# elrodrigues/deneva-plus

Measured on AMD Instinct MI355X. Metric: committed txns/sec (node) YCSB zipf0.9 at 1/2/4/8 GPUs; abort-set bit-exact, higher is better.
Workload: dtype u64; 1 GPU; YCSB config D: 16,777,216 rows/partition, 1,048,576-txn epoch in total; cc_alg=NO_WAIT, rows_per_partition=16777216, txns_per_epoch=1048576, txns_per_epoch_per_gpu=1048576, req_per_query=10, parallelism=1 GPU, decision_lanes=4, sequence_order=one origin

## Files before the change

deneva-plus_amd/csrc/dvcc_common.h:

```cpp
#pragma once
#include "dvcc_internal.h"

namespace dvcc {

__device__ __forceinline__ uint32_t mask_rank(uint64_t mask) {
    return __builtin_amdgcn_mbcnt_hi((uint32_t)(mask >> 32),
                                     __builtin_amdgcn_mbcnt_lo((uint32_t)mask, 0u));
}

__device__ __forceinline__ uint64_t match_digit(uint32_t d, uint64_t valid) {
    uint64_t peers = valid;
#pragma unroll
    for (int b = 0; b < kRadixBits; b++) {
        const uint32_t bit = (d >> b) & 1u;
        const uint64_t m = __ballot(bit);
        peers &= bit ? m : ~m;
    }
    return peers;
}

__device__ __forceinline__ uint32_t block_excl_scan256(uint32_t v, uint32_t *lds4, uint32_t *total) {
    const uint32_t lane = threadIdx.x & 63, wave = threadIdx.x >> 6;
    uint32_t x = v;
#pragma unroll
// ... 256 lines not shown
    } else {
        for (uint32_t j = t.bstart[bk], end = t.bstart[bk + 1]; j < end; j++) {
            const IxEntry e = t.ix[j];
            if (e.key == key) { row = e.row; found = true; break; }
        }
    }
    if (!found) {
        if (miss) *miss = true;
        else set_err(ctr, ERRB_KEY);
    }
    row += t.row_base;
    return found;
}

template <bool DENSE>
__device__ __forceinline__ bool kk_row(const KillKeys &kk, uint64_t key, uint64_t &row, Counters *ctr) {
    if constexpr (DENSE) {
        row = key + kk.dense_base;
        if (key < kk.dense_lim) return true;
        set_err(ctr, ERRB_KEY);
        return false;
    } else {
        return probe_row(kk.tabs.t[0], kk.tabs.n > 0, key, row, ctr);
    }
}

__device__ __forceinline__ uint32_t row_word(const uint32_t *__restrict__ acc_row, const RecRows &rr, uint64_t a) {
    if (rr.on && !rr.recs)
        return (uint32_t)(rr.keys[a] + rr.dense_base) | (rr.types[a] == DV_WR ? AR_WR : 0u);
    const uint32_t w = (rr.on ? rr.recs : acc_row)[a];
    return ((w & ~AR_WR) + (rr.on ? (uint32_t)rr.dense_base : 0u)) | (w & AR_WR);
}

}
```

deneva-plus_amd/csrc/dvcc_kernels.hip:

```cpp
#include <hip/hip_ext.h>

#include "dvcc_common.h"
#include "dvcc_tpcc.h"

#ifndef DVCC_PROBE_HIST_WAVES
#define DVCC_PROBE_HIST_WAVES 6
#endif

namespace dvcc {


constexpr int kPV = 4;
template <bool HIST, bool RSV>
__device__ __forceinline__ void probe_body(const Tables &tabs, const uint64_t *__restrict__ keys,
                                           const uint32_t *__restrict__ keys32,
                                                  const uint8_t *__restrict__ types,
                                                  const uint32_t *__restrict__ acc_txn,
                                                  const uint8_t *__restrict__ tables, uint64_t n,
                                                  uint32_t n_txn, uint32_t slog,
                                                  uint64_t *__restrict__ pairs,
                                                  uint32_t *__restrict__ tb_start,
                                                  uint32_t *__restrict__ tb_end,
                                                  uint8_t *__restrict__ tlen,
                                                  uint32_t *__restrict__ acc_row, Counters *ctr,
// ... 271 lines not shown
                              acc_txn, tables, n_acc, n_txn, slog, pairs, tb_start, tb_end, tlen, acc_row, ctr,
                              counts, ntiles, ts, rsv_cols);
    else if (counts)
        DV_LAUNCH_EV(k_probe_hist<false>, blocks, kBlock, 0, s, ev0, ev1, tabs, keys, keys32, types,
                              acc_txn, tables, n_acc, n_txn, slog, pairs, tb_start, tb_end, tlen, acc_row, ctr,
                              counts, ntiles, ts, nullptr);
    else if (rsv_cols)
        DV_LAUNCH_EV(k_probe<true>, blocks, kBlock, 0, s, ev0, ev1, tabs, keys, keys32, types, acc_txn,
                              tables, n_acc, n_txn, slog, pairs, tb_start, tb_end, tlen, acc_row, ctr, lim, ts, n_dev,
                              rsv_cols);
    else
        DV_LAUNCH_EV(k_probe<false>, blocks, kBlock, 0, s, ev0, ev1, tabs, keys, keys32, types, acc_txn,
                              tables, n_acc, n_txn, slog, pairs, tb_start, tb_end, tlen, acc_row, ctr, lim, ts, n_dev,
                              nullptr);
}

__global__ __launch_bounds__(kBlock) void k_probe_tb(Tables tabs, const uint64_t *__restrict__ keys,
                                                     const uint8_t *__restrict__ types,
                                                     const uint32_t *__restrict__ recs,
                                                     const uint32_t *__restrict__ txn_begin, uint64_t n_acc,
                                                     uint32_t n_txn, uint32_t K, uint32_t slog,
                                                     uint64_t *__restrict__ pairs, uint8_t *__restrict__ tlen,
                                                     uint32_t *__restrict__ acc_row, Counters *ctr,
                                                     const uint64_t *__restrict__ ts,
                                                     const uint32_t *__restrict__ n_acc_dev) {
    if (n_acc_dev && (uint64_t)*n_acc_dev < n_acc) n_acc = *n_acc_dev;
    if (blockIdx.x == 0 && threadIdx.x == 0) {
        ctr->n_acc = (uint32_t)n_acc;
        const uint64_t ak = txn_begin[K];
        ctr->a_acc = (uint32_t)(ak < n_acc ? ak : n_acc);
        if (txn_begin[0] != 0u || txn_begin[n_txn] != n_acc) set_err(ctr, ERRB_TXN);
    }
    bool bad = false, big_seen = false, ts_bad = false;
    for (uint32_t t = blockIdx.x * kBlock + threadIdx.x; t < n_txn; t += gridDim.x * kBlock) {
        const uint32_t a0 = txn_begin[t], a1 = txn_begin[t + 1];
        if (a1 < a0 || a1 > n_acc) {
            bad = true;
            continue;
        }
        const uint32_t len = a1 - a0;
        const bool big = len > (1u << slog);
        big_seen |= big;
        if (ts && t > 0 && ts[t] <= ts[t - 1]) ts_bad = true;
        if (t >= K) continue;
        tlen[t] = (uint8_t)(big ? (1u << slog) : len);
        constexpr uint32_t kU = 8;
        for (uint32_t j0 = 0; j0 < len; j0 += kU) {
            uint64_t key[kU];
            uint32_t wrs[kU];
            const KillKeys kk{tabs, keys, types, recs, 0, 0};
#pragma unroll
            for (uint32_t j = 0; j < kU; j++) {
                wrs[j] = 0;
                key[j] = j0 + j < len ? kk_key(kk, a0 + j0 + j, wrs[j]) : 0ull;
            }
#pragma unroll
            for (uint32_t j = 0; j < kU; j++) {
                if (j0 + j >= len) break;
                uint64_t row = 0;
                probe_row(tabs.t[0], tabs.n > 0, key[j], row, ctr);
                const uint32_t wr = wrs[j];
                const uint32_t pos = j0 + j;
                if (acc_row) acc_row[a0 + pos] = (uint32_t)row | (wr ? AR_WR : 0u);
                pairs[a0 + pos] = pair_pack(row, t, (pos >> slog) ? 0u : pos, wr);
            }
        }
    }
    if (bad) set_err(ctr, ERRB_TXN);
    if (big_seen) set_err(ctr, ERRB_BIG);
    if (ts_bad) set_err(ctr, ERRB_TS);
}

void launch_probe_tb(hipStream_t s, const Tables &tabs, const uint64_t *keys, const uint8_t *types,
                     const uint32_t *recs, const uint32_t *txn_begin, uint64_t n_acc, uint32_t n_txn, uint32_t K,
                     uint32_t slog, uint64_t *pairs, uint8_t *tlen, uint32_t *acc_row, Counters *ctr,
                     const uint64_t *ts, hipEvent_t ev0, hipEvent_t ev1, const uint32_t *n_acc_dev) {
#ifndef DVCC_PROBE_TB_GRID
#define DVCC_PROBE_TB_GRID 4096
#endif
    uint32_t g = (n_txn + kBlock - 1) / kBlock;
    g = g < 1 ? 1 : (g > DVCC_PROBE_TB_GRID ? DVCC_PROBE_TB_GRID : g);
    DV_LAUNCH_EV(k_probe_tb, g, kBlock, 0, s, ev0, ev1, tabs, keys, types, recs, txn_begin, n_acc, n_txn, K, slog,
                 pairs, tlen, acc_row, ctr, ts, n_acc_dev);
}


__device__ __forceinline__ uint64_t sort_n(uint64_t n, const uint32_t *n_dev) {
    return n_dev && (uint64_t)*n_dev < n ? (uint64_t)*n_dev : n;
}

__device__ __forceinline__ uint32_t row_hash(uint64_t key, uint32_t hmul, int hbits) {
    return ((uint32_t)(key >> 32) * hmul) & ((1u << hbits) - 1u);
}
template <int W>
__device__ __forceinline__ uint32_t key_digit(uint64_t key, int shift, uint32_t hmul, int hbits) {
    return hmul ? row_hash(key, hmul, hbits) >> (hbits - W) : (uint32_t)(key >> shift) & ((1u << W) - 1u);
}

// ... 26 lines not shown
        } else if (valid) {
            atomicAdd(&wc[wave][d], 1u);
        }
    }
    __syncthreads();
    for (uint32_t d = tid; d < kRadix; d += kBlock)
        counts[(uint64_t)d * nblocks + blockIdx.x] = wc[0][d] + wc[1][d] + wc[2][d] + wc[3][d];
}

__global__ __launch_bounds__(kBlock) void k_radix_scan(uint32_t *__restrict__ counts, uint32_t nblocks,
                                                       uint32_t *__restrict__ digit_tot,
                                                       const uint32_t *__restrict__ n_dev) {
    __shared__ uint32_t lds4[4];
    uint32_t *c = counts + (uint64_t)blockIdx.x * nblocks;
    if (n_dev && nblocks_for(*n_dev) < nblocks) nblocks = nblocks_for(*n_dev);
    const uint32_t tot = block_chunk_scan256(c, nblocks, lds4);
    if (threadIdx.x == 0) digit_tot[blockIdx.x] = tot;
}

__global__ __launch_bounds__(kBlock) void k_radix_scatter(
    const uint64_t *__restrict__ in, uint64_t *__restrict__ out, uint64_t n, int shift, const uint32_t *__restrict__ counts,
    const uint32_t *__restrict__ digit_tot, uint32_t nblocks, const uint32_t *__restrict__ n_dev,
    uint32_t hmul, int hbits, uint32_t *__restrict__ digit_pre) {
    __shared__ __attribute__((aligned(16))) uint64_t skeys[kTile];
    n = sort_n(n, n_dev);
    if ((uint64_t)blockIdx.x * kTile >= n) return;
    __shared__ uint32_t wc[4][kRadix];
    __shared__ uint32_t dstart[kRadix];
    __shared__ uint64_t gbase[kRadix];
    __shared__ uint32_t lds4[4];
    const uint32_t tid = threadIdx.x, lane = tid & 63, wave = tid >> 6;
    const uint64_t tile0 = (uint64_t)blockIdx.x * kTile;

    {
        const uint32_t d = tid;
        const uint32_t dex = block_excl_scan256(digit_tot[d], lds4, nullptr);
        if (digit_pre && blockIdx.x == 0) digit_pre[d] = dex;
        gbase[d] = (uint64_t)dex + counts[(uint64_t)d * nblocks + blockIdx.x];
        for (int w = 0; w < 4; w++) wc[w][d] = 0;
    }
    __syncthreads();

    const uint64_t base = tile0 + wave * (64 * kIPT);
    uint64_t k[kIPT];
    uint32_t r[kIPT];
#pragma unroll
    for (int j = 0; j < kIPT; j++) {
        const uint64_t idx = base + j * 64 + lane;
        k[j] = idx < n ? in[idx] : 0;
    }
#pragma unroll
    for (int j = 0; j < kIPT; j++) {
        const uint64_t idx = base + j * 64 + lane;
        const bool valid = idx < n;
        const uint32_t d = key_digit<kRadixBits>(k[j], shift, hmul, hbits);
        const uint64_t vmask = __ballot(valid);
        const uint64_t peers = match_digit(d, vmask);
        const uint32_t before = wc[wave][d];
        r[j] = before + mask_rank(peers);
        if (valid && lane == (uint32_t)__builtin_ctzll(peers)) wc[wave][d] = before + (uint32_t)__popcll(peers);
    }
    __syncthreads();
    {
        const uint32_t d = tid;
        const uint32_t c0 = wc[0][d], c1 = wc[1][d], c2 = wc[2][d], c3 = wc[3][d];
        wc[0][d] = 0;
        wc[1][d] = c0;
        wc[2][d] = c0 + c1;
        wc[3][d] = c0 + c1 + c2;
        const uint32_t ds = block_excl_scan256(c0 + c1 + c2 + c3, lds4, nullptr);
        dstart[d] = ds;
        gbase[d] -= ds;
    }
    __syncthreads();
#pragma unroll
    for (int j = 0; j < kIPT; j++) {
        const uint64_t idx = base + j * 64 + lane;
        if (idx < n) {
            const uint32_t d = key_digit<kRadixBits>(k[j], shift, hmul, hbits);
            const uint32_t pos = dstart[d] + wc[wave][d] + r[j];
            skeys[pos] = k[j];
        }
    }
    __syncthreads();
    const uint32_t tile_n = (uint32_t)((n - tile0) < (uint64_t)kTile ? (n - tile0) : kTile);
    for (uint32_t p = tid; p < tile_n; p += kBlock) {
        const uint64_t key = skeys[p];
// ... 26 lines not shown
    for (int j = 0; j < kIPT; j++) {
        const uint64_t idx = base + j * 64 + lane;
        const bool valid = idx < n;
        const uint32_t d = key_digit<W>(k[j], shift, hmul, hbits);
        const uint32_t d0 = __builtin_amdgcn_readfirstlane(d);
        const uint64_t vmask = __ballot(valid);
        if (__ballot(valid && d == d0) == vmask) {
            if (lane == 0) wc[wave][d0] += (uint32_t)__popcll(vmask);
        } else if (valid) {
            atomicAdd(&wc[wave][d], 1u);
        }
    }
    __syncthreads();
    for (uint32_t d = tid; d < R; d += kBlock)
        counts[(uint64_t)d * nblocks + blockIdx.x] = wc[0][d] + wc[1][d] + wc[2][d] + wc[3][d];
}

template <int W>
__global__ __launch_bounds__(kBlock) void k_radix_scatter_w(const uint64_t *__restrict__ in, uint64_t *__restrict__ out,
                                                            uint64_t n, int shift, const uint32_t *__restrict__ counts,
                                                            const uint32_t *__restrict__ digit_tot, uint32_t nblocks,
                                                            const uint32_t *__restrict__ n_dev, uint32_t hmul,
                                                            int hbits, uint32_t *__restrict__ digit_pre) {
    constexpr uint32_t R = 1u << W, PER = R / kBlock;
    __shared__ __attribute__((aligned(16))) uint64_t skeys[kTile];
    __shared__ uint32_t wc[4][R];
    __shared__ uint32_t dstart[R];
    __shared__ uint32_t gbase[R];
    __shared__ uint32_t lds4[4];
    n = sort_n(n, n_dev);
    if ((uint64_t)blockIdx.x * kTile >= n) return;
    const uint32_t tid = threadIdx.x, lane = tid & 63, wave = tid >> 6;
    const uint64_t tile0 = (uint64_t)blockIdx.x * kTile;
    {
        uint32_t t[PER], sum = 0;
#pragma unroll
        for (uint32_t q = 0; q < PER; q++) {
            t[q] = digit_tot[tid * PER + q];
            sum += t[q];
        }
        uint32_t pre = block_excl_scan256(sum, lds4, nullptr);
#pragma unroll
        for (uint32_t q = 0; q < PER; q++) {
            const uint32_t d = tid * PER + q;
            if (digit_pre && blockIdx.x == 0) digit_pre[d] = pre;
            gbase[d] = pre + counts[(uint64_t)d * nblocks + blockIdx.x];
            pre += t[q];
            wc[0][d] = wc[1][d] = wc[2][d] = wc[3][d] = 0;
        }
    }
    __syncthreads();
    const uint64_t base = tile0 + wave * (64 * kIPT);
    uint64_t k[kIPT];
    uint32_t r[kIPT];
#pragma unroll
    for (int j = 0; j < kIPT; j++) {
        const uint64_t idx = base + j * 64 + lane;
        k[j] = idx < n ? in[idx] : 0;
    }
#pragma unroll
    for (int j = 0; j < kIPT; j++) {
        const uint64_t idx = base + j * 64 + lane;
        const bool valid = idx < n;
        const uint32_t d = key_digit<W>(k[j], shift, hmul, hbits);
        uint64_t peers = __ballot(valid);
#pragma unroll
        for (int b = 0; b < W; b++) {
            const uint32_t bit = (d >> b) & 1u;
            const uint64_t m = __ballot(bit);
            peers &= bit ? m : ~m;
        }
        const uint32_t before = wc[wave][d];
        r[j] = before + mask_rank(peers);
        if (valid && lane == (uint32_t)__builtin_ctzll(peers)) wc[wave][d] = before + (uint32_t)__popcll(peers);
    }
    __syncthreads();
    {
        uint32_t tot[PER], sum = 0;
#pragma unroll
        for (uint32_t q = 0; q < PER; q++) {
            const uint32_t d = tid * PER + q;
            const uint32_t c0 = wc[0][d], c1 = wc[1][d], c2 = wc[2][d], c3 = wc[3][d];
            wc[0][d] = 0;
            wc[1][d] = c0;
            wc[2][d] = c0 + c1;
            wc[3][d] = c0 + c1 + c2;
            tot[q] = c0 + c1 + c2 + c3;
            sum += tot[q];
        }
        uint32_t ds = block_excl_scan256(sum, lds4, nullptr);
#pragma unroll
        for (uint32_t q = 0; q < PER; q++) {
            const uint32_t d = tid * PER + q;
            dstart[d] = ds;
            gbase[d] -= ds;
            ds += tot[q];
// ... 250 lines not shown
            const uint32_t d = valid ? ((row_hash(src[i], hmul, hbits) & hmask) >> sh) & (kRadix - 1) : 0u;
            const uint32_t d0 = __builtin_amdgcn_readfirstlane(d);
            const uint64_t vm = __ballot(valid);
            if (__ballot(valid && d == d0) == vm) {
                if (lane == 0 && vm) atomicAdd(&tot[d0], (uint32_t)__popcll(vm));
            } else if (valid) {
                atomicAdd(&tot[d], 1u);
            }
        }
        __syncthreads();
        if (tid < 64) {
            uint32_t v[4], s4 = 0;
#pragma unroll
            for (int q = 0; q < 4; q++) {
                v[q] = tot[4 * lane + q];
                s4 += v[q];
            }
            uint32_t pre = wave_incl_sum(s4, lane) - s4;
#pragma unroll
            for (int q = 0; q < 4; q++) {
                run[4 * lane + q] = pre;
                pre += v[q];
            }
        }
        __syncthreads();
        for (uint32_t c0 = 0; c0 < m; c0 += kChunk) {
            const uint32_t mc = m - c0 < kChunk ? m - c0 : kChunk;
            const uint32_t steps = (mc + kBucketThreads - 1) / kBucketThreads;
            for (uint32_t d = lane; d < (uint32_t)kRadix; d += 64) wc[wave][d] = 0;
            uint64_t k[kBucketGroup];
            uint32_t r[kBucketGroup];
#pragma unroll
            for (int s = 0; s < kBucketGroup; s++) {
                if ((uint32_t)s < steps) {
                    const uint32_t e = (wave * steps + s) * 64 + lane;
                    const bool valid = e < mc;
                    k[s] = valid ? src[c0 + e] : 0ull;
                    r[s] = bucket_rank(((row_hash(k[s], hmul, hbits) & hmask) >> sh) & (kRadix - 1), valid,
                                       wc[wave], lane);
                }
            }
            __syncthreads();
            bucket_bases(wc, tot, run);
#pragma unroll
            for (int s = 0; s < kBucketGroup; s++) {
                if ((uint32_t)s < steps) {
                    const uint32_t e = (wave * steps + s) * 64 + lane;
                    if (e < mc) dst[wc[wave][((row_hash(k[s], hmul, hbits) & hmask) >> sh) & (kRadix - 1)] + r[s]] = k[s];
                }
            }
            __syncthreads();
        }
    }
    if (!(passes & 1)) {
        for (uint32_t i = tid; i < m; i += kBucketThreads) B[i] = A[i];
    }
}

int radix_sort_rows(hipStream_t s, uint64_t *pairs[2], uint64_t n, int key_bits, uint32_t *counts,
                    uint32_t *digit_tot, hipEvent_t *scatter_ev, bool hist0_done, const uint32_t *n_dev,
                    bool lsd_only) {
    if (n == 0) return 0;
    const uint32_t nb = nblocks_for(n);
    int cur = 0, pass = 0;
    if (!lsd_only && bucket_sort_applies(n, key_bits, hist0_done, n_dev != nullptr)) {
        const int lo = kBucketLoBits(key_bits);
        const uint32_t hmul = kRowHashMul;
        uint32_t *digit_pre = digit_tot + kRadixMax;
        hipEvent_t e0 = scatter_ev ? scatter_ev[0] : nullptr, e1 = scatter_ev ? scatter_ev[1] : nullptr;
        if (lo == 9)
// ... 599 lines not shown
```

deneva-plus_amd/csrc/dvcc_prefix.hip:

```cpp
#include <algorithm>

#include "dvcc_common.h"

namespace dvcc {

namespace {
#ifndef DVCC_KILL_IPT
#define DVCC_KILL_IPT 2
#endif
constexpr int kKillIPT = DVCC_KILL_IPT;
constexpr uint32_t kKillTile = kBlock * kKillIPT;
constexpr uint32_t RS_RD = 1u, RS_WR = 2u;

__device__ __forceinline__ uint32_t row_bits(const uint32_t *rs, uint32_t row) {
    return (rs[row >> 4] >> ((row & 15u) * 2u)) & 3u;
}
}

#ifndef DVCC_HOT_LOG
#define DVCC_HOT_LOG 16
#endif
#ifndef DVCC_BLOOM_LOG
#define DVCC_BLOOM_LOG 20
#endif
constexpr uint32_t kHotRows = 1u << DVCC_HOT_LOG, kHotWords = kHotRows / 16;
constexpr uint32_t kBloomBits = 1u << DVCC_BLOOM_LOG, kBloomWords = kBloomBits / 32;
static_assert((kHotWords + kBloomWords) * sizeof(uint32_t) <= 160u * 1024u,
              "k_kill's hot row words + Bloom filter exceed gfx950's 160 KiB of LDS per workgroup");
__device__ __forceinline__ uint32_t bloom_bit(uint32_t row) { return (row * 0x9E3779B1u) >> (32 - DVCC_BLOOM_LOG); }

uint64_t row_state_words(uint64_t rows) {
    return std::max<uint64_t>(((rows + 15) / 16 + 3) & ~3ull, kHotWords) + kBloomWords;
}

#ifndef DVCC_MARK_BLOCK
#define DVCC_MARK_BLOCK 512
#endif
constexpr int kMarkBlock = DVCC_MARK_BLOCK;
__global__ __launch_bounds__(kMarkBlock) void k_prefix_mark(uint8_t *__restrict__ status,
                                                            const uint32_t *__restrict__ tb_start,
                                                            const uint32_t *__restrict__ tb_end,
                                                            const uint32_t *__restrict__ acc_row, RecRows rr,
                                                            uint32_t K, uint32_t *__restrict__ row_state,
                                                            uint64_t state_words,
                                                            uint32_t *__restrict__ bloom, int nowait,
                                                            Counters *__restrict__ ctr,
                                                            const uint32_t *__restrict__ words) {
    __shared__ uint32_t s_hot[kHotWords];
    if (input_err(ctr)) return;
    if (ctr->halt) {
        if (blockIdx.x == 0 && threadIdx.x == 0) ctr->a_halt = 1u;
        return;
    }
    if (blockIdx.x == 0 && threadIdx.x == 0) {
        const uint32_t r0 = ctr->async_wr0 ? ctr->async_wr0 : ctr->async_r0;
        ctr->a_rounds = r0 ? r0 + ctr->async_iters : 1u;
    }
    for (uint32_t i = threadIdx.x; i < kHotWords; i += kMarkBlock) s_hot[i] = 0;
    __syncthreads();
    uint32_t und = 0;
    for (uint32_t t = blockIdx.x * kMarkBlock + threadIdx.x; t < K; t += gridDim.x * kMarkBlock) {
        if (words) {
            const uint8_t st = word_status(words[t]);
            status[t] = st;
            und += st == ST_UNDEC ? 1u : 0u;
            if (st != ST_COMMIT) continue;
        } else if (status[t] != ST_COMMIT) {
            continue;
        }
        constexpr uint32_t kMU = 8;
        for (uint32_t a0 = tb_start[t], e = tb_end[t]; a0 < e; a0 += kMU) {
            uint32_t arw[kMU];
#pragma unroll
            for (uint32_t u = 0; u < kMU; u++) arw[u] = a0 + u < e ? row_word(acc_row, rr, a0 + u) : 0u;
#pragma unroll
            for (uint32_t u = 0; u < kMU; u++) {
                if (a0 + u >= e) continue;
                const uint32_t ar = arw[u];
                const uint32_t row = ar & ~AR_WR;
                const uint32_t bit = (ar & AR_WR) ? RS_WR : (nowait ? RS_RD : 0u);
                if (!bit) continue;
                if (row < kHotRows) {
                    atomicOr(&s_hot[row >> 4], bit << ((row & 15u) * 2u));
                } else {
                    atomicOr(&row_state[row >> 4], bit << ((row & 15u) * 2u));
                    const uint32_t h = bloom_bit(row);
                    atomicOr(&bloom[h >> 5], 1u << (h & 31u));
                }
            }
        }
    }
    if (und) {
        set_err(ctr, ERRB_SPIN);
        atomicMax(&ctr->spin_site, 2u);
    }
    __syncthreads();
    for (uint32_t i = threadIdx.x; i < kHotWords && i < state_words; i += kMarkBlock) {
        const uint32_t w = s_hot[i];
        if (w) atomicOr(&row_state[i], w);
    }
}

#ifndef DVCC_KILL_WORDS
#define DVCC_KILL_WORDS 8
#endif
constexpr int kKillWords = DVCC_KILL_WORDS;
constexpr int kKillBlock = 1024;
#ifndef DVCC_KILL_GRID
#define DVCC_KILL_GRID 256
// ... 208 lines not shown
        info[t - K] = killed ? 0u : len | 0x80000000u;
        cnt += killed ? 0u : 1u;
        acc += len;
    }
    uint32_t tc = 0, ta = 0;
    (void)block_excl_scan256(cnt, lds4, &tc);
    (void)block_excl_scan256(acc, lds4, &ta);
    if (tid == 0) {
        tsum[2 * blockIdx.x] = tc;
        tsum[2 * blockIdx.x + 1] = ta;
    }
}

template <int KEYS>
__global__ __launch_bounds__(kBlock) void k_kill_emit(
    const uint32_t *__restrict__ tb_start, const uint32_t *__restrict__ tb_end, uint32_t *__restrict__ acc_row,
    uint32_t K, uint32_t n_txn,
    const uint64_t *__restrict__ skip_bits, const uint32_t *__restrict__ info, const uint32_t *__restrict__ tsum,
    uint32_t *__restrict__ map,
    uint8_t *__restrict__ status_b, uint8_t *__restrict__ tlen_b, uint64_t *__restrict__ pairs_b, Counters *ctr,
    KillKeys kk, const uint32_t *__restrict__ row_state, int nowait) {
    __shared__ Agg wt_c[kBlock / 64], wt_a[kBlock / 64], wt_f[kBlock / 64];
    __shared__ uint32_t s_sub0, s_ab0, s_nsurv, s_nacc, s_nfull;
    __shared__ uint32_t l_a0[kKillTile], l_pre[kKillTile + 1];
    __shared__ uint32_t l_st[kKillTile], l_len[kKillTile];
    __shared__ uint32_t l_end[KEYS ? kKillTile : 1], l_fl[KEYS ? kKillTile : 1], l_skip[KEYS ? kKillTile : 1];
    __shared__ uint32_t l_fpre[KEYS == 1 ? kKillTile + 1 : 1];
    const uint32_t m = n_txn > K ? n_txn - K : 0u;
    const uint32_t ntiles = (m + kKillTile - 1) / kKillTile;
    if (blockIdx.x >= ntiles || input_err(ctr) || ctr->halt) return;
    const uint32_t tid = threadIdx.x, lane = tid & 63, wave = tid >> 6;
    const uint32_t tile = blockIdx.x;
    const uint32_t t_lo = K + tile * kKillTile;
#pragma unroll
    for (int j = 0; j < kKillIPT; j++) {
        const uint32_t t = t_lo + j * kBlock + tid;
        l_st[j * kBlock + tid] = t < n_txn ? tb_start[t] : 0u;
        l_len[j * kBlock + tid] = t < n_txn ? info[t - K] : 0u;
        if constexpr (KEYS) l_end[j * kBlock + tid] = t < n_txn ? tb_end[t] : 0u;
    }
    if (wave < 2) {
        uint32_t sum = 0;
        for (uint32_t q0 = 0; q0 < tile; q0 += 8 * 64) {
            uint32_t v[8];
#pragma unroll
            for (uint32_t u = 0; u < 8; u++) {
                const uint32_t q = q0 + u * 64 + lane;
                v[u] = q < tile ? tsum[2 * q + wave] : 0u;
            }
#pragma unroll
            for (uint32_t u = 0; u < 8; u++) sum += v[u];
        }
#pragma unroll
        for (int off = 32; off > 0; off >>= 1) sum += __shfl_xor(sum, off, 64);
        if (lane == 0) {
            (wave == 0 ? s_sub0 : s_ab0) = sum;
            if (tile == ntiles - 1) (wave == 0 ? ctr->b_txn : ctr->b_acc) = sum + tsum[2 * tile + wave];
        }
    }
    __syncthreads();
    const uint32_t first = t_lo + tid * kKillIPT;
    uint32_t surv = 0, cnt = 0, acc = 0, full = 0;
    uint32_t a0s[kKillIPT], lens[kKillIPT], fls[kKillIPT];
#pragma unroll
    for (int j = 0; j < kKillIPT; j++) {
        const uint32_t w = l_len[tid * kKillIPT + j];
        a0s[j] = l_st[tid * kKillIPT + j];
        lens[j] = w & 0x7FFFFFFFu;
        fls[j] = KEYS ? l_end[tid * kKillIPT + j] - a0s[j] : 0u;
        if (!w) continue;
        surv |= 1u << j;
        cnt++;
// ... 41 lines not shown
        l_a0[ls] = a0s[j];
        l_pre[ls] = la;
        if constexpr (KEYS) l_fl[ls] = fls[j];
        if constexpr (KEYS == 1) {
            l_fpre[ls] = lf;
            l_skip[ls] = 0;
        }
        if constexpr (KEYS == 2)
            l_skip[ls] = skip_bits && fls[j] <= 32u ? range_field(skip_bits, a0s[j], a0s[j] + fls[j]) : 0u;
        la += lens[j];
        lf += fls[j];
        ls++;
    }
    if (tid == 0) {
        l_pre[s_nsurv] = s_nacc;
        if constexpr (KEYS == 1) l_fpre[s_nsurv] = s_nfull;
    }
    __syncthreads();
    if constexpr (KEYS == 1) {
        constexpr uint32_t kU = 4;
        const uint32_t ns = s_nsurv, nf = s_nfull;
        for (uint32_t g0 = 0; g0 < nf; g0 += kBlock * kU) {
            uint32_t a[kU], wr[kU];
            uint64_t key[kU];
#pragma unroll
            for (uint32_t u = 0; u < kU; u++) {
                const uint32_t g = g0 + u * kBlock + tid;
                uint32_t lo = 0, hi = ns;
                while (hi - lo > 1) {
                    const uint32_t mid = (lo + hi) >> 1;
                    if (l_fpre[mid] <= g) lo = mid;
                    else hi = mid;
                }
                a[u] = l_a0[lo] + (g - l_fpre[lo]);
                wr[u] = 0;
                key[u] = g < nf ? kk_key(kk, a[u], wr[u]) : 0ull;
            }
            uint32_t rows[kU];
#pragma unroll
            for (uint32_t u = 0; u < kU; u++) {
                uint64_t row = 0;
                if (g0 + u * kBlock + tid < nf)
                    kk_row<false>(kk, key[u], row, ctr);
                rows[u] = (uint32_t)row;
            }
#pragma unroll
            for (uint32_t u = 0; u < kU; u++) {
                const uint32_t g = g0 + u * kBlock + tid;
                if (g >= nf) continue;
                acc_row[a[u]] = rows[u] | (wr[u] ? AR_WR : 0u);
#ifdef DVCC_EMIT_ROW_STATE
                const bool skip = nowait && !wr[u] && row_bits(row_state, rows[u]) == RS_RD;
#else
                const bool skip = skip_bits && ((skip_bits[a[u] >> 6] >> (a[u] & 63u)) & 1ull) != 0;
#endif
                if (skip) {
                    uint32_t lo = 0, hi = ns;
                    while (hi - lo > 1) {
                        const uint32_t mid = (lo + hi) >> 1;
                        if (l_fpre[mid] <= g) lo = mid;
                        else hi = mid;
                    }
                    if (l_fpre[lo + 1] - l_fpre[lo] <= 32u) atomicOr(&l_skip[lo], 1u << (g - l_fpre[lo]));
                }
            }
        }
        __syncthreads();
    }
    constexpr uint32_t kCompactU = 4;
    const uint32_t ns = s_nsurv, na = s_nacc, ab0 = s_ab0;
    for (uint32_t g0 = 0; g0 < na; g0 += kBlock * kCompactU) {
        uint32_t sv[kCompactU], qv[kCompactU], ar[kCompactU];
#pragma unroll
        for (uint32_t u = 0; u < kCompactU; u++) {
            const uint32_t g = g0 + u * kBlock + tid;
            uint32_t lo = 0, hi = ns;
            while (hi - lo > 1) {
                const uint32_t mid = (lo + hi) >> 1;
                if (l_pre[mid] <= g) lo = mid;
                else hi = mid;
            }
            sv[u] = lo;
            qv[u] = g - l_pre[lo];
            uint32_t a = 0;
            if (g < na) {
                if constexpr (KEYS) {
                    if (l_fl[lo] <= 32u) {
                        uint32_t kept = ~l_skip[lo];
                        for (uint32_t r = qv[u]; r; r--) kept &= kept - 1;
                        a = l_a0[lo] + (uint32_t)__builtin_ctz(kept);
                    } else {
                        a = skip_bits ? nth_kept(skip_bits, l_a0[lo], qv[u]) : l_a0[lo] + qv[u];
                    }
                } else {
                    a = skip_bits ? nth_kept(skip_bits, l_a0[lo], qv[u]) : l_a0[lo] + qv[u];
                }
            }
            if constexpr (KEYS) {
                uint64_t row = 0;
                uint32_t w = 0;
                if (g < na) kk_row<KEYS == 2>(kk, kk_key(kk, a, w), row, ctr);
                ar[u] = g < na ? (uint32_t)row | (w ? AR_WR : 0u) : 0u;
            } else {
                ar[u] = g < na ? acc_row[a] : 0u;
            }
        }
#pragma unroll
        for (uint32_t u = 0; u < kCompactU; u++) {
            const uint32_t g = g0 + u * kBlock + tid;
            if (g < na) pairs_b[ab0 + g] = pair_pack(ar[u] & ~AR_WR, sub0 + sv[u], qv[u], ar[u] >> 31);
        }
    }
}

__global__ __launch_bounds__(kBlock) void k_sub_scatter_back(const uint32_t *__restrict__ map,
                                                             const uint8_t *__restrict__ status_b,
                                                             uint8_t *__restrict__ status, Counters *ctr,
                                                             const uint32_t *__restrict__ words) {
    if (input_err(ctr) || ctr->halt) return;
    const uint32_t S = ctr->b_txn;
    uint32_t und = 0;
    for (uint32_t i = blockIdx.x * kBlock + threadIdx.x; i < S; i += gridDim.x * kBlock) {
        const uint8_t st = words ? word_status(words[i]) : status_b[i];
        status[map[i]] = st;
        und += st == ST_UNDEC ? 1u : 0u;
    }
    if (und) {
        set_err(ctr, ERRB_SPIN);
        atomicMax(&ctr->spin_site, 2u);
    }
}

namespace {
uint32_t grid_of(uint64_t n, uint32_t cap) {
    const uint64_t g = (n + kBlock - 1) / kBlock;
    return (uint32_t)(g < 1 ? 1 : (g > cap ? cap : g));
}
}
// ... 56 lines not shown
```

deneva-plus_amd/csrc/dvcc_rounds.hip:

```cpp
#include <hip/hip_ext.h>

#include "dvcc_common.h"

namespace dvcc {

namespace {

constexpr uint32_t B_CA = 1u, B_UA = 2u, B_CW = 4u, B_UW = 8u, B_KEEP = 16u;
constexpr uint32_t kCarryHead = 1u << 31;
constexpr uint32_t kCarryInit = B_UA | B_UW | B_KEEP | kCarryHead;
constexpr uint8_t VB_OK = 1, VB_ABORT = 2;
constexpr uint32_t F_WR = 1u, F_HEAD = 2u, F_DONE = 4u;

template <class E>
__device__ __forceinline__ uint32_t r_txn(E e, uint32_t slog) {
    return (uint32_t)(e >> (slog + 3));
}

template <class E>
__device__ __forceinline__ uint32_t elem_value(E e, uint8_t s, int nowait) {
    const bool wr = (e & F_WR) != 0;
    if (s == ST_COMMIT) return (nowait ? B_CA : 0u) | (wr ? B_CW : 0u);
    if (s == ST_UNDEC) return (nowait ? B_UA : 0u) | (wr ? B_UW : 0u);
    return 0u;
}

template <bool ALL = false, class E>
__device__ __forceinline__ E decide_elem(E e, uint32_t excl, int nowait, uint8_t *__restrict__ vb8,
                                         uint32_t slog, uint8_t *status) {
    if (e & F_DONE) return e;
    const uint32_t sel = (nowait && (e & F_WR)) ? (excl & (B_CA | B_UA)) : ((excl >> 2) & (B_CA | B_UA));
    if (sel & B_CA) {
        status[r_txn(e, slog)] = ST_ABORT;
// ... 113 lines not shown
#define DVCC_ROUND_T64 1024
#endif
#ifndef DVCC_ROUND_IPT64
#define DVCC_ROUND_IPT64 4
#endif
struct Geo {
    static constexpr int kThreads = sizeof(EIn) == 4 ? 1024 : DVCC_ROUND_T64;
    static constexpr int kMinWaves = sizeof(EIn) == 4 ? 4 : 3;
    static constexpr int kWaves = kThreads / 64;
    static constexpr int kIPT = sizeof(EIn) == 4 ? DVCC_ROUND_IPT : DVCC_ROUND_IPT64;
    static constexpr uint32_t kTile = kThreads * kIPT;
    static_assert(kTile >= (uint32_t)kRTile, "round tiles at least kRTile elements");
};
__device__ __forceinline__ uint32_t pad16(uint32_t j) { return j + (j >> 4); }

template <class EIn>
struct TileLds {
    EIn el[Geo<EIn>::kTile + Geo<EIn>::kTile / 16];
    EIn next;
    uint64_t prev;
    Agg wt[Geo<EIn>::kWaves];
    RAgg rw[Geo<EIn>::kWaves];
    Agg pre;
    uint32_t tot;
    uint32_t gpos;
};

template <class EIn>
__device__ __forceinline__ void load_tile(const EIn *__restrict__ src, uint32_t base, uint32_t tile_n,
                                          uint32_t n, EIn *s, EIn *s_next, EIn past_end) {
    constexpr int V = 16 / sizeof(EIn);
    constexpr int T = Geo<EIn>::kThreads;
    const uint32_t tid = threadIdx.x;
#pragma unroll
    for (int q = 0; q < Geo<EIn>::kIPT / V; q++) {
        const uint32_t j = (q * T + tid) * V;
        if (j + V <= tile_n) {
            if constexpr (V == 2) {
                const ulonglong2 x = *reinterpret_cast<const ulonglong2 *>(src + base + j);
                s[pad16(j)] = x.x;
                s[pad16(j + 1)] = x.y;
            } else {
                const uint4 x = *reinterpret_cast<const uint4 *>(src + base + j);
                s[pad16(j)] = x.x;
                s[pad16(j + 1)] = x.y;
                s[pad16(j + 2)] = x.z;
                s[pad16(j + 3)] = x.w;
            }
        } else {
            for (int k = 0; k < V; k++)
                if (j + k < tile_n) s[pad16(j + k)] = src[base + j + k];
        }
    }
    if (tid == 0) *s_next = base + tile_n < n ? src[base + tile_n] : past_end;
}

template <bool FIRST, class EIn, class E>
__device__ __forceinline__ void round_tile(TileLds<EIn> &sh, uint32_t tile, uint32_t n, uint32_t ntiles,
                                           const EIn *__restrict__ el_in, E *__restrict__ el_out,
                                           uint32_t *__restrict__ n_out, uint8_t *status,
                                           uint8_t *__restrict__ vb8, uint32_t slog, int nowait,
                                           uint64_t *desc, uint32_t tag, uint32_t *und_reset,
                                           Counters *ctr);

__device__ __forceinline__ void reset_und(uint32_t *und_reset, Counters *ctr) {
    if (und_reset) *und_reset = 0;
    else for (int k = 0; k < kSlots; k++) ctr->slot[k].undecided = 0;
}

template <bool FIRST, class EIn, class E>
__device__ __forceinline__ void round_tile(TileLds<EIn> &sh, uint32_t tile, uint32_t n, uint32_t ntiles,
                                           const EIn *__restrict__ el_in, E *__restrict__ el_out,
                                           uint32_t *__restrict__ n_out, uint8_t *status,
                                           uint8_t *__restrict__ vb8, uint32_t slog, int nowait,
                                           uint64_t *desc, uint32_t tag, uint32_t *und_reset,
                                           Counters *ctr) {
    using G = Geo<EIn>;
    constexpr int IPT = G::kIPT;
    const uint32_t tid = threadIdx.x, lane = tid & 63, wave = tid >> 6;
    const uint32_t base = tile * G::kTile;
    const uint32_t tile_n = n - base < G::kTile ? n - base : G::kTile;
    load_tile<EIn>(el_in, base, tile_n, n, sh.el, &sh.next, FIRST ? (EIn)~0ull : (EIn)F_HEAD);
    if (FIRST && tid == 0) sh.prev = base > 0 ? (uint64_t)el_in[base - 1] : ~0ull;
    __syncthreads();

    const uint32_t first = tid * IPT;
    const int cnt = first >= tile_n ? 0 : (tile_n - first < (uint32_t)IPT ? (int)(tile_n - first) : IPT);
    E e[IPT];
    uint32_t v[IPT];
    uint32_t nhm = 0;
    uint32_t tmask = 0;
    if constexpr (FIRST) {
        uint64_t pp = first == 0 ? sh.prev : (uint64_t)sh.el[pad16(first - 1)];
        const uint64_t pn = first + IPT < tile_n ? (uint64_t)sh.el[pad16(first + IPT)] : (uint64_t)sh.next;
        uint64_t p[IPT];
#pragma unroll
        for (int j = 0; j < IPT; j++) p[j] = j < cnt ? (uint64_t)sh.el[pad16(first + j)] : ~0ull;
#pragma unroll
        for (int j = 0; j < IPT; j++) {
            e[j] = (E)F_HEAD;
            if (j < cnt) {
                const bool head = pair_row(pp) != pair_row(p[j]);
                const uint64_t q = j + 1 < cnt ? p[j + 1] : (cnt < IPT ? ~0ull : pn);
                const bool rep = !head && pair_txn(pp) == pair_txn(p[j]);
                uint32_t wr = (uint32_t)(p[j] & 1u);
                const uint64_t id = ((uint64_t)pair_txn(p[j]) << slog) | pair_pos(p[j]);
                if (rep) {
                    tmask |= 1u << j;
                    vb8[id] = VB_OK;
                    if (nowait && ((p[j] | pp) & 1u)) status[pair_txn(p[j])] = ST_ABORT;
                } else if ((q >> 8) == (p[j] >> 8)) {
                    for (uint32_t k = base + first + j + 1; k < n && !wr; k++) {
                        const uint64_t x = (uint64_t)el_in[k];
                        if ((x >> 8) != (p[j] >> 8)) break;
                        wr |= (uint32_t)(x & 1u);
                    }
// ... 98 lines not shown
        ctr->nund[0] = n_txn_dev ? *n_txn_dev : n_txn0;
        ctr->async_go = 0;
        ctr->async_r0 = 0;
        ctr->async_wr0 = 0;
        ctr->async_iters = 0;
        ctr->async_block = 0;
    }
    const uint32_t n = und && !input_err(ctr) ? n_live : 0u;
    const uint32_t ntiles = (n + Geo<EIn>::kTile - 1) / Geo<EIn>::kTile;
    if (blockIdx.x == 0 && threadIdx.x == 0) {
        if (round < (uint32_t)kRoundLog && (und || round == 0)) {
            ctr->log_live[round] = n_live;
            ctr->log_und[round] = und_in ? und : 0u;
        }
        if (n) ctr->pass_live += n;
    }
    const bool publisher = pub && threadIdx.x == 0 && blockIdx.x == (ntiles ? ntiles - 1 : 0);
    if (blockIdx.x >= ntiles) {
        if (ntiles == 0 && blockIdx.x == 0 && threadIdx.x == 0) { *n_out = 0; reset_und(und_reset, ctr); }
    } else {
        if (threadIdx.x == 0) s_tile = atomicAdd(tile_ctr, 1u);
        __syncthreads();
        round_tile<FIRST, EIn, E>(sh, s_tile, n, ntiles, el_in, el_out, n_out, status, vb8, slog,
                                  nowait, desc, tag, und_reset, ctr);
    }
    if (publisher) {
        __hip_atomic_store(&pub->le, ((unsigned long long)n_live << 32) | ctr->err | ctr->peer_err,
                           __ATOMIC_RELAXED, __HIP_MEMORY_SCOPE_SYSTEM);
        __hip_atomic_store(&pub->ru, ((unsigned long long)round << 32) | und, __ATOMIC_RELAXED,
                           __HIP_MEMORY_SCOPE_SYSTEM);
    }
}

__device__ __forceinline__ uint8_t txn_verdict(const uint8_t *__restrict__ v, uint32_t len, uint32_t *n_ok = nullptr) {
    uint32_t any_abort = 0, all_ok = 1, ok = 0;
    for (uint32_t w = 0; w < len; w += 16) {
        const uint4 x4 = *reinterpret_cast<const uint4 *>(v + w);
        const uint32_t x[4] = {x4.x, x4.y, x4.z, x4.w};
#pragma unroll
        for (uint32_t q = 0; q < 4; q++) {
            const int nb = (int)len - (int)(w + 4 * q);
            const uint32_t m = nb >= 4 ? 0xFFFFFFFFu : (nb <= 0 ? 0u : (1u << (8 * nb)) - 1u);
            any_abort |= x[q] & 0x02020202u & m;
            all_ok &= (x[q] & m) == (0x01010101u & m);
            if (n_ok) ok += __popc(x[q] & 0x01010101u & m);
        }
    }
    if (n_ok) *n_ok = ok;
    return any_abort ? V_ABORT : (all_ok ? 0 : V_WAIT);
}

#ifndef DVCC_SETTLE_IPT
#define DVCC_SETTLE_IPT 1
#endif
constexpr uint32_t kSettleIPT = DVCC_SETTLE_IPT, kSettleChunk = kBlock * kSettleIPT;

__device__ __forceinline__ bool settle_txn(uint8_t *__restrict__ status, const uint8_t *__restrict__ vb8,
                                           uint32_t slog, const uint8_t *__restrict__ tlen,
                                           uint32_t t, uint32_t *__restrict__ tword = nullptr) {
    const uint8_t s0 = status[t];
    if (s0 != ST_UNDEC) {
        if (tword) tword[t] = s0 | ((uint32_t)tlen[t] << 16);
        return false;
    }
    const uint32_t len = tlen[t];
    uint32_t ok = 0;
    const uint8_t v = txn_verdict(vb8 + ((size_t)t << slog), len, tword ? &ok : nullptr);
    const uint8_t s = (v & V_ABORT) ? ST_ABORT : (!(v & V_WAIT) ? ST_COMMIT : ST_UNDEC);
    if (s != ST_UNDEC) status[t] = s;
    if (tword) tword[t] = s | ((s == ST_UNDEC ? ok : 0u) << 8) | (len << 16);
    return s == ST_UNDEC;
}

struct SettleLds {
    uint32_t keep[kSettleChunk];
    uint32_t cnt, base;
};

template <bool FIRST>
__device__ __forceinline__ void settle_chunk(SettleLds &sh, uint32_t lo, uint32_t n,
                                             uint8_t *__restrict__ status,
                                             const uint8_t *__restrict__ vb8, uint32_t slog,
                                             const uint8_t *__restrict__ tlen,
                                             const uint32_t *__restrict__ list_in,
                                             uint32_t *__restrict__ list_out,
                                             uint32_t *__restrict__ n_out,
                                             uint32_t *__restrict__ tword = nullptr) {
    if (threadIdx.x == 0) sh.cnt = 0;
    __syncthreads();
    const uint32_t lane = threadIdx.x & 63;
#pragma unroll
    for (uint32_t k = 0; k < kSettleIPT; k++) {
        const uint32_t i = lo + k * kBlock + threadIdx.x;
        uint32_t t = 0;
        bool keep = false;
        if (i < n) {
            t = FIRST ? i : list_in[i];
            keep = settle_txn(status, vb8, slog, tlen, t, tword);
        }
        const uint64_t m = __ballot(keep);
// ... 826 lines not shown
```

Before: 178.2 million committed txns/s.

## Batch and hoist independent global loads across probe, sort, mark, kill and settle kernels

Restructures several kernels so independent global loads are issued together before they are used. The probe loop software-prefetches the next transaction's bounds and timestamps. Radix scatter loads its keys before the digit scan, and mark, kill and compact batch their key and type gathers with clamped indices. Round tile loads take a vectorized full-tile path, and settle loads the first verdict vector speculatively. The aim is more memory-level parallelism and less exposed latency, at the cost of extra registers and some redundant loads at clamped indices.

```diff
diff --git a/deneva-plus_amd/csrc/dvcc_common.h b/deneva-plus_amd/csrc/dvcc_common.h
--- a/deneva-plus_amd/csrc/dvcc_common.h
+++ b/deneva-plus_amd/csrc/dvcc_common.h
@@ -312,4 +312,27 @@
     return ((w & ~AR_WR) + (rr.on ? (uint32_t)rr.dense_base : 0u)) | (w & AR_WR);
 }
 
-}
+template <uint32_t N>
+__device__ __forceinline__ void row_words(const uint32_t *__restrict__ acc_row, const RecRows &rr,
+                                          const uint32_t (&idx)[N], uint32_t (&out)[N]) {
+    if (rr.on && !rr.recs) {
+        uint64_t k[N];
+        uint8_t ty[N];
+#pragma unroll
+        for (uint32_t u = 0; u < N; u++) {
+            k[u] = rr.keys[idx[u]];
+            ty[u] = rr.types[idx[u]];
+        }
+#pragma unroll
+        for (uint32_t u = 0; u < N; u++) out[u] = (uint32_t)(k[u] + rr.dense_base) | (ty[u] == DV_WR ? AR_WR : 0u);
+        return;
+    }
+    const uint32_t *__restrict__ src = rr.on ? rr.recs : acc_row;
+    const uint32_t add = rr.on ? (uint32_t)rr.dense_base : 0u;
+#pragma unroll
+    for (uint32_t u = 0; u < N; u++) out[u] = src[idx[u]];
+#pragma unroll
+    for (uint32_t u = 0; u < N; u++) out[u] = ((out[u] & ~AR_WR) + add) | (out[u] & AR_WR);
+}
+
+}
diff --git a/deneva-plus_amd/csrc/dvcc_kernels.hip b/deneva-plus_amd/csrc/dvcc_kernels.hip
--- a/deneva-plus_amd/csrc/dvcc_kernels.hip
+++ b/deneva-plus_amd/csrc/dvcc_kernels.hip
@@ -327,27 +327,35 @@
         if (txn_begin[0] != 0u || txn_begin[n_txn] != n_acc) set_err(ctr, ERRB_TXN);
     }
     bool bad = false, big_seen = false, ts_bad = false;
-    for (uint32_t t = blockIdx.x * kBlock + threadIdx.x; t < n_txn; t += gridDim.x * kBlock) {
-        const uint32_t a0 = txn_begin[t], a1 = txn_begin[t + 1];
+    auto one_txn = [&](uint32_t t, uint32_t a0, uint32_t a1, uint64_t ts1, uint64_t ts0) {
         if (a1 < a0 || a1 > n_acc) {
             bad = true;
-            continue;
+            return;
         }
         const uint32_t len = a1 - a0;
         const bool big = len > (1u << slog);
         big_seen |= big;
-        if (ts && t > 0 && ts[t] <= ts[t - 1]) ts_bad = true;
-        if (t >= K) continue;
+        if (ts && t > 0 && ts1 <= ts0) ts_bad = true;
+        if (t >= K) return;
         tlen[t] = (uint8_t)(big ? (1u << slog) : len);
         constexpr uint32_t kU = 8;
         for (uint32_t j0 = 0; j0 < len; j0 += kU) {
             uint64_t key[kU];
             uint32_t wrs[kU];
-            const KillKeys kk{tabs, keys, types, recs, 0, 0};
-#pragma unroll
-            for (uint32_t j = 0; j < kU; j++) {
-                wrs[j] = 0;
-                key[j] = j0 + j < len ? kk_key(kk, a0 + j0 + j, wrs[j]) : 0ull;
+            if (recs) {
+#pragma unroll
+                for (uint32_t j = 0; j < kU; j++) {
+                    const uint32_t r = recs[j0 + j < len ? a0 + j0 + j : a1 - 1];
+                    wrs[j] = r >> 31;
+                    key[j] = r & 0x7FFFFFFFu;
+                }
+            } else {
+#pragma unroll
+                for (uint32_t j = 0; j < kU; j++) {
+                    const uint32_t i = j0 + j < len ? a0 + j0 + j : a1 - 1;
+                    key[j] = keys[i];
+                    wrs[j] = types[i] == DV_WR ? 1u : 0u;
+                }
             }
 #pragma unroll
             for (uint32_t j = 0; j < kU; j++) {
@@ -359,6 +367,25 @@
                 if (acc_row) acc_row[a0 + pos] = (uint32_t)row | (wr ? AR_WR : 0u);
                 pairs[a0 + pos] = pair_pack(row, t, (pos >> slog) ? 0u : pos, wr);
             }
+        }
+    };
+    const uint32_t stride = gridDim.x * kBlock;
+    uint32_t t = blockIdx.x * kBlock + threadIdx.x;
+    if (t < n_txn) {
+        uint32_t a0 = txn_begin[t], a1 = txn_begin[t + 1];
+        uint64_t ts1 = ts ? ts[t] : 0ull, ts0 = ts ? ts[t > 0 ? t - 1 : 0u] : 0ull;
+        for (;;) {
+            const bool more = n_txn - t > stride;
+            const uint32_t tn = more ? t + stride : t;
+            const uint32_t na0 = txn_begin[tn], na1 = txn_begin[tn + 1];
+            const uint64_t nts1 = ts ? ts[tn] : 0ull, nts0 = ts ? ts[tn > 0 ? tn - 1 : 0u] : 0ull;
+            one_txn(t, a0, a1, ts1, ts0);
+            if (!more) break;
+            t = tn;
+            a0 = na0;
+            a1 = na1;
+            ts1 = nts1;
+            ts0 = nts0;
         }
     }
     if (bad) set_err(ctr, ERRB_TXN);
@@ -451,27 +478,29 @@
     const uint32_t tid = threadIdx.x, lane = tid & 63, wave = tid >> 6;
     const uint64_t tile0 = (uint64_t)blockIdx.x * kTile;
 
-    {
-        const uint32_t d = tid;
-        const uint32_t dex = block_excl_scan256(digit_tot[d], lds4, nullptr);
-        if (digit_pre && blockIdx.x == 0) digit_pre[d] = dex;
-        gbase[d] = (uint64_t)dex + counts[(uint64_t)d * nblocks + blockIdx.x];
-        for (int w = 0; w < 4; w++) wc[w][d] = 0;
-    }
-    __syncthreads();
-
     const uint64_t base = tile0 + wave * (64 * kIPT);
     uint64_t k[kIPT];
     uint32_t r[kIPT];
 #pragma unroll
     for (int j = 0; j < kIPT; j++) {
         const uint64_t idx = base + j * 64 + lane;
-        k[j] = idx < n ? in[idx] : 0;
-    }
+        k[j] = in[idx < n ? idx : n - 1];
+    }
+    {
+        const uint32_t d = tid;
+        const uint32_t dtot = digit_tot[d], dcnt = counts[(uint64_t)d * nblocks + blockIdx.x];
+        const uint32_t dex = block_excl_scan256(dtot, lds4, nullptr);
+        if (digit_pre && blockIdx.x == 0) digit_pre[d] = dex;
+        gbase[d] = (uint64_t)dex + dcnt;
+        for (int w = 0; w < 4; w++) wc[w][d] = 0;
+    }
+    __syncthreads();
+
 #pragma unroll
     for (int j = 0; j < kIPT; j++) {
         const uint64_t idx = base + j * 64 + lane;
         const bool valid = idx < n;
+        k[j] = valid ? k[j] : 0;
         const uint32_t d = key_digit<kRadixBits>(k[j], shift, hmul, hbits);
         const uint64_t vmask = __ballot(valid);
         const uint64_t peers = match_digit(d, vmask);
@@ -564,36 +593,39 @@
     if ((uint64_t)blockIdx.x * kTile >= n) return;
     const uint32_t tid = threadIdx.x, lane = tid & 63, wave = tid >> 6;
     const uint64_t tile0 = (uint64_t)blockIdx.x * kTile;
+    const uint64_t base = tile0 + wave * (64 * kIPT);
+    uint64_t k[kIPT];
+    uint32_t r[kIPT];
+#pragma unroll
+    for (int j = 0; j < kIPT; j++) {
+        const uint64_t idx = base + j * 64 + lane;
+        k[j] = in[idx < n ? idx : n - 1];
+    }
     {
-        uint32_t t[PER], sum = 0;
+        uint32_t t[PER], c[PER], sum = 0;
 #pragma unroll
         for (uint32_t q = 0; q < PER; q++) {
             t[q] = digit_tot[tid * PER + q];
-            sum += t[q];
-        }
+            c[q] = counts[(uint64_t)(tid * PER + q) * nblocks + blockIdx.x];
+        }
+#pragma unroll
+        for (uint32_t q = 0; q < PER; q++) sum += t[q];
         uint32_t pre = block_excl_scan256(sum, lds4, nullptr);
 #pragma unroll
         for (uint32_t q = 0; q < PER; q++) {
             const uint32_t d = tid * PER + q;
             if (digit_pre && blockIdx.x == 0) digit_pre[d] = pre;
-            gbase[d] = pre + counts[(uint64_t)d * nblocks + blockIdx.x];
+            gbase[d] = pre + c[q];
             pre += t[q];
             wc[0][d] = wc[1][d] = wc[2][d] = wc[3][d] = 0;
         }
     }
     __syncthreads();
-    const uint64_t base = tile0 + wave * (64 * kIPT);
-    uint64_t k[kIPT];
-    uint32_t r[kIPT];
-#pragma unroll
-    for (int j = 0; j < kIPT; j++) {
-        const uint64_t idx = base + j * 64 + lane;
-        k[j] = idx < n ? in[idx] : 0;
-    }
 #pragma unroll
     for (int j = 0; j < kIPT; j++) {
         const uint64_t idx = base + j * 64 + lane;
         const bool valid = idx < n;
+        k[j] = valid ? k[j] : 0;
         const uint32_t d = key_digit<W>(k[j], shift, hmul, hbits);
         uint64_t peers = __ballot(valid);
 #pragma unroll
@@ -910,10 +942,15 @@
             uint32_t r[kBucketGroup];
 #pragma unroll
             for (int s = 0; s < kBucketGroup; s++) {
+                const uint32_t e = (wave * steps + s) * 64 + lane;
+                k[s] = src[c0 + ((uint32_t)s < steps && e < mc ? e : 0u)];
+            }
+#pragma unroll
+            for (int s = 0; s < kBucketGroup; s++) {
                 if ((uint32_t)s < steps) {
                     const uint32_t e = (wave * steps + s) * 64 + lane;
                     const bool valid = e < mc;
-                    k[s] = valid ? src[c0 + e] : 0ull;
+                    k[s] = valid ? k[s] : 0ull;
                     r[s] = bucket_rank(((row_hash(k[s], hmul, hbits) & hmask) >> sh) & (kRadix - 1), valid,
                                        wc[wave], lane);
                 }
diff --git a/deneva-plus_amd/csrc/dvcc_prefix.hip b/deneva-plus_amd/csrc/dvcc_prefix.hip
--- a/deneva-plus_amd/csrc/dvcc_prefix.hip
+++ b/deneva-plus_amd/csrc/dvcc_prefix.hip
@@ -14,6 +14,30 @@
 
 __device__ __forceinline__ uint32_t row_bits(const uint32_t *rs, uint32_t row) {
     return (rs[row >> 4] >> ((row & 15u) * 2u)) & 3u;
+}
+
+template <uint32_t N>
+__device__ __forceinline__ void kk_keys(const KillKeys &kk, const uint32_t (&a)[N], uint64_t (&key)[N],
+                                        uint32_t (&wr)[N]) {
+    if (kk.recs) {
+        uint32_t r[N];
+#pragma unroll
+        for (uint32_t u = 0; u < N; u++) r[u] = kk.recs[a[u]];
+#pragma unroll
+        for (uint32_t u = 0; u < N; u++) {
+            wr[u] = r[u] >> 31;
+            key[u] = r[u] & 0x7FFFFFFFu;
+        }
+        return;
+    }
+    uint8_t ty[N];
+#pragma unroll
+    for (uint32_t u = 0; u < N; u++) {
+        key[u] = kk.keys[a[u]];
+        ty[u] = kk.types[a[u]];
+    }
+#pragma unroll
+    for (uint32_t u = 0; u < N; u++) wr[u] = ty[u] == DV_WR ? 1u : 0u;
 }
 }
 
@@ -60,6 +84,8 @@
     __syncthreads();
     uint32_t und = 0;
     for (uint32_t t = blockIdx.x * kMarkBlock + threadIdx.x; t < K; t += gridDim.x * kMarkBlock) {
+        uint32_t a0 = tb_start[t];
+        const uint32_t e = tb_end[t];
         if (words) {
             const uint8_t st = word_status(words[t]);
             status[t] = st;
@@ -68,13 +94,14 @@
         } else if (status[t] != ST_COMMIT) {
             continue;
         }
-        constexpr uint32_t kMU = 8;
-        for (uint32_t a0 = tb_start[t], e = tb_end[t]; a0 < e; a0 += kMU) {
-            uint32_t arw[kMU];
-#pragma unroll
-            for (uint32_t u = 0; u < kMU; u++) arw[u] = a0 + u < e ? row_word(acc_row, rr, a0 + u) : 0u;
-#pragma unroll
-            for (uint32_t u = 0; u < kMU; u++) {
+        constexpr uint32_t kMU = 8, kMStep = 2 * kMU;
+        for (; a0 < e; a0 += kMStep) {
+            uint32_t arw[kMStep], ai[kMStep];
+#pragma unroll
+            for (uint32_t u = 0; u < kMStep; u++) ai[u] = a0 + u < e ? a0 + u : e - 1;
+            row_words<kMStep>(acc_row, rr, ai, arw);
+#pragma unroll
+            for (uint32_t u = 0; u < kMStep; u++) {
                 if (a0 + u >= e) continue;
                 const uint32_t ar = arw[u];
                 const uint32_t row = ar & ~AR_WR;
@@ -349,12 +376,23 @@
     const uint32_t tid = threadIdx.x, lane = tid & 63, wave = tid >> 6;
     const uint32_t tile = blockIdx.x;
     const uint32_t t_lo = K + tile * kKillTile;
-#pragma unroll
-    for (int j = 0; j < kKillIPT; j++) {
-        const uint32_t t = t_lo + j * kBlock + tid;
-        l_st[j * kBlock + tid] = t < n_txn ? tb_start[t] : 0u;
-        l_len[j * kBlock + tid] = t < n_txn ? info[t - K] : 0u;
-        if constexpr (KEYS) l_end[j * kBlock + tid] = t < n_txn ? tb_end[t] : 0u;
+    {
+        uint32_t st[kKillIPT], inf[kKillIPT], en[kKillIPT];
+#pragma unroll
+        for (int j = 0; j < kKillIPT; j++) {
+            const uint32_t t = t_lo + j * kBlock + tid;
+            const uint32_t tc = t < n_txn ? t : n_txn - 1;
+            st[j] = tb_start[tc];
+            inf[j] = info[tc - K];
+            en[j] = KEYS ? tb_end[tc] : 0u;
+        }
+#pragma unroll
+        for (int j = 0; j < kKillIPT; j++) {
+            const bool in = t_lo + j * kBlock + tid < n_txn;
+            l_st[j * kBlock + tid] = in ? st[j] : 0u;
+            l_len[j * kBlock + tid] = in ? inf[j] : 0u;
+            if constexpr (KEYS) l_end[j * kBlock + tid] = in ? en[j] : 0u;
+        }
     }
     if (wave < 2) {
         uint32_t sum = 0;
@@ -462,10 +500,10 @@
                     if (l_fpre[mid] <= g) lo = mid;
                     else hi = mid;
                 }
-                a[u] = l_a0[lo] + (g - l_fpre[lo]);
+                a[u] = g < nf ? l_a0[lo] + (g - l_fpre[lo]) : 0u;
                 wr[u] = 0;
-                key[u] = g < nf ? kk_key(kk, a[u], wr[u]) : 0ull;
-            }
+            }
+            kk_keys<kU>(kk, a, key, wr);
             uint32_t rows[kU];
 #pragma unroll
             for (uint32_t u = 0; u < kU; u++) {
@@ -500,7 +538,7 @@
     constexpr uint32_t kCompactU = 4;
     const uint32_t ns = s_nsurv, na = s_nacc, ab0 = s_ab0;
     for (uint32_t g0 = 0; g0 < na; g0 += kBlock * kCompactU) {
-        uint32_t sv[kCompactU], qv[kCompactU], ar[kCompactU];
+        uint32_t sv[kCompactU], qv[kCompactU], ar[kCompactU], av[kCompactU];
 #pragma unroll
         for (uint32_t u = 0; u < kCompactU; u++) {
             const uint32_t g = g0 + u * kBlock + tid;
@@ -526,14 +564,22 @@
                     a = skip_bits ? nth_kept(skip_bits, l_a0[lo], qv[u]) : l_a0[lo] + qv[u];
                 }
             }
-            if constexpr (KEYS) {
+            av[u] = a;
+        }
+        if constexpr (KEYS) {
+            uint64_t key[kCompactU];
+            uint32_t w[kCompactU];
+            kk_keys<kCompactU>(kk, av, key, w);
+#pragma unroll
+            for (uint32_t u = 0; u < kCompactU; u++) {
                 uint64_t row = 0;
-                uint32_t w = 0;
-                if (g < na) kk_row<KEYS == 2>(kk, kk_key(kk, a, w), row, ctr);
-                ar[u] = g < na ? (uint32_t)row | (w ? AR_WR : 0u) : 0u;
-            } else {
-                ar[u] = g < na ? acc_row[a] : 0u;
-            }
+                const bool in = g0 + u * kBlock + tid < na;
+                if (in) kk_row<KEYS == 2>(kk, key[u], row, ctr);
+                ar[u] = in ? (uint32_t)row | (w[u] ? AR_WR : 0u) : 0u;
+            }
+        } else {
+#pragma unroll
+            for (uint32_t u = 0; u < kCompactU; u++) ar[u] = acc_row[av[u]];
         }
 #pragma unroll
         for (uint32_t u = 0; u < kCompactU; u++) {
diff --git a/deneva-plus_amd/csrc/dvcc_rounds.hip b/deneva-plus_amd/csrc/dvcc_rounds.hip
--- a/deneva-plus_amd/csrc/dvcc_rounds.hip
+++ b/deneva-plus_amd/csrc/dvcc_rounds.hip
@@ -1,4 +1,6 @@
 #include <hip/hip_ext.h>
+
+#include <type_traits>
 
 #include "dvcc_common.h"
 
@@ -178,6 +180,26 @@
     constexpr int V = 16 / sizeof(EIn);
     constexpr int T = Geo<EIn>::kThreads;
     const uint32_t tid = threadIdx.x;
+    const EIn nxt = src[base + tile_n < n ? base + tile_n : n - 1];
+    if (tile_n == Geo<EIn>::kTile) {
+        constexpr int Q = Geo<EIn>::kIPT / V;
+        using Vec = typename std::conditional<V == 2, ulonglong2, uint4>::type;
+        Vec x[Q];
+#pragma unroll
+        for (int q = 0; q < Q; q++) x[q] = *reinterpret_cast<const Vec *>(src + base + (q * T + tid) * V);
+#pragma unroll
+        for (int q = 0; q < Q; q++) {
+            const uint32_t j = (q * T + tid) * V;
+            s[pad16(j)] = x[q].x;
+            s[pad16(j + 1)] = x[q].y;
+            if constexpr (V == 4) {
+                s[pad16(j + 2)] = x[q].z;
+                s[pad16(j + 3)] = x[q].w;
+            }
+        }
+        if (tid == 0) *s_next = base + tile_n < n ? nxt : past_end;
+        return;
+    }
 #pragma unroll
     for (int q = 0; q < Geo<EIn>::kIPT / V; q++) {
         const uint32_t j = (q * T + tid) * V;
@@ -198,7 +220,7 @@
                 if (j + k < tile_n) s[pad16(j + k)] = src[base + j + k];
         }
     }
-    if (tid == 0) *s_next = base + tile_n < n ? src[base + tile_n] : past_end;
+    if (tid == 0) *s_next = base + tile_n < n ? nxt : past_end;
 }
 
 template <bool FIRST, class EIn, class E>
@@ -226,8 +248,10 @@
     const uint32_t tid = threadIdx.x, lane = tid & 63, wave = tid >> 6;
     const uint32_t base = tile * G::kTile;
     const uint32_t tile_n = n - base < G::kTile ? n - base : G::kTile;
+    uint64_t prv = 0;
+    if constexpr (FIRST) prv = (uint64_t)el_in[base > 0 ? base - 1 : 0u];
     load_tile<EIn>(el_in, base, tile_n, n, sh.el, &sh.next, FIRST ? (EIn)~0ull : (EIn)F_HEAD);
-    if (FIRST && tid == 0) sh.prev = base > 0 ? (uint64_t)el_in[base - 1] : ~0ull;
+    if (FIRST && tid == 0) sh.prev = base > 0 ? prv : ~0ull;
     __syncthreads();
 
     const uint32_t first = tid * IPT;
@@ -392,10 +416,11 @@
     }
 }
 
-__device__ __forceinline__ uint8_t txn_verdict(const uint8_t *__restrict__ v, uint32_t len, uint32_t *n_ok = nullptr) {
+__device__ __forceinline__ uint8_t txn_verdict(const uint8_t *__restrict__ v, uint32_t len, uint32_t *n_ok = nullptr,
+                                               const uint4 *first = nullptr) {
     uint32_t any_abort = 0, all_ok = 1, ok = 0;
     for (uint32_t w = 0; w < len; w += 16) {
-        const uint4 x4 = *reinterpret_cast<const uint4 *>(v + w);
+        const uint4 x4 = first && w == 0 ? *first : *reinterpret_cast<const uint4 *>(v + w);
         const uint32_t x[4] = {x4.x, x4.y, x4.z, x4.w};
 #pragma unroll
         for (uint32_t q = 0; q < 4; q++) {
@@ -419,13 +444,15 @@
                                            uint32_t slog, const uint8_t *__restrict__ tlen,
                                            uint32_t t, uint32_t *__restrict__ tword = nullptr) {
     const uint8_t s0 = status[t];
+    const uint32_t len = tlen[t];
+    uint4 v0 = *reinterpret_cast<const uint4 *>(vb8 + ((size_t)t << slog));
+    asm volatile("" : "+v"(v0.x), "+v"(v0.y), "+v"(v0.z), "+v"(v0.w));
     if (s0 != ST_UNDEC) {
-        if (tword) tword[t] = s0 | ((uint32_t)tlen[t] << 16);
+        if (tword) tword[t] = s0 | (len << 16);
         return false;
     }
-    const uint32_t len = tlen[t];
     uint32_t ok = 0;
-    const uint8_t v = txn_verdict(vb8 + ((size_t)t << slog), len, tword ? &ok : nullptr);
+    const uint8_t v = txn_verdict(vb8 + ((size_t)t << slog), len, tword ? &ok : nullptr, &v0);
     const uint8_t s = (v & V_ABORT) ? ST_ABORT : (!(v & V_WAIT) ? ST_COMMIT : ST_UNDEC);
     if (s != ST_UNDEC) status[t] = s;
     if (tword) tword[t] = s | ((s == ST_UNDEC ? ok : 0u) << 8) | (len << 16);
```

Measured after the change: 178.8 million committed txns/s (median of 2 runs). No clear change (+0.3%).
